# zzuiekongning/MGDT-YOLO

Measured on AMD Instinct MI355X. Metric: images/sec @640x640 bs=32 per GPU, detection forward + NMS (whole job: 1 GPU(s)), higher is better.
Workload: dtype bf16; 1 GPU; mspa_c2f_gd_yolov8-n (MSPA-C2f + GD neck + Detect, nc=80) 640x640 inference, batch 32/GPU: forward + decode + NMS(conf 0.25, iou 0.7), hipGraph replay, 4 batches in flight (one captured graph per resident batch, replayed round-robin on 4 streams); global_batch=32, parallelism=replicas x1 (batch-sharded, no data-path collective), rccl_ranks=1, input=bfloat16 NCHW images, 8 different batches resident in HBM (600 MiB) cycled, detections_last_step=9600, weights=seeded random init (no checkpoints offline), batches_in_flight=4

## Files before the change

mgdt_yolo_amd/csrc/pointwise.hip:

```cpp
#include <algorithm>
#include <vector>

#include <type_traits>
#include "common.h"

#define SPR_SPLITS 16

static inline int grid_for(long work, int block = 256, int cap = 8192) { return (int)std::min<long>((work + block - 1) / block, cap); }

struct PixIdx { FastDiv fq, fw, fh; int Q, W, H; };
static inline PixIdx make_pixidx(int H, int W, int Q) { return PixIdx{make_fastdiv((uint32_t)Q), make_fastdiv((uint32_t)W), make_fastdiv((uint32_t)H), Q, W, H}; }
__device__ __forceinline__ void decode_idx(uint32_t i, const PixIdx& d, int& n, int& h, int& w, int& q) {
  uint32_t t = fdiv(i, d.fq);
  q = (int)(i - t * d.Q);
  uint32_t t2 = fdiv(t, d.fw);
  w = (int)(t - t2 * d.W);
  uint32_t t3 = fdiv(t2, d.fh);
  h = (int)(t2 - t3 * d.H);
  n = (int)t3;
}
template <typename T, int V> __device__ __forceinline__ void ldv(const T* p, float (&v)[V]) {
#pragma unroll
  for (int k = 0; k < V; k += 4) {
    f32x4 t = load4<T>(p + k);
// ... 399 lines not shown
    for (int hj = 0; hj < hid; ++hj) s = fmaf(w2s[ci * r2 + hj], hbuf[gi * hid + hj], s);
    obuf[o] = 1.f / (1.f + expf(-s));
  }
  __syncthreads();
  SPR_STAMP();
  for (int ci = tid; ci < cw; ci += 256) {
    float mx = -INFINITY;
    for (int gi = 0; gi < G; ++gi) mx = fmaxf(mx, obuf[gi * cw + ci]);
    float den = 0.f;
    for (int gi = 0; gi < G; ++gi) { const float e = expf(obuf[gi * cw + ci] - mx); att[gi * cw + ci] = e; den += e; }
    for (int gi = 0; gi < G; ++gi) att[gi * cw + ci] /= den;
  }
  __syncthreads();
}

template <typename T, int V>
__global__ __launch_bounds__(256) void spr_attn_scale_kernel(const float* __restrict__ partial, const float* __restrict__ w1, const float* __restrict__ b1,
                                                             const float* __restrict__ w2, const float* __restrict__ b2, int C, int G, int H, int W,
                                                             const T* __restrict__ x, long xsn, long xsh, long xsw, T* __restrict__ y, long ysn, long ysh,
                                                             long ysw, FastDiv fd_q, FastDiv fd_w, int nsplit, int tiles_x, int tiles_y, SprPool pa, SprPool pb, FastDiv fd_gst,
                                                             FastDiv fd_tx, FastDiv fd_l4, int fast, unsigned long long* dbg) {
  extern __shared__ float sm[];
  unsigned long long TS[10]; int nt = 0;
  auto stamp = [&]() __attribute__((always_inline)) { if (dbg) TS[nt++] = __builtin_amdgcn_s_memrealtime(); };
  stamp();
  const int n = blockIdx.y, cw = C / G, hid = cw / 4;
  float* pooled = sm;
  float* hbuf = sm + C * 5;
  float* obuf = hbuf + G * hid;
  float* att = obuf + C;
  const int hs1 = bin_start(1, H, 2), he0 = bin_end(0, H, 2), ws1 = bin_start(1, W, 2), we0 = bin_end(0, W, 2);
  const float cnt[5] = {(float)H * W, (float)he0 * we0, (float)he0 * (W - ws1), (float)(H - hs1) * we0, (float)(H - hs1) * (W - ws1)};
  __shared__ float red[5 * 256];
  if (fast) {
    spr_prologue_fast(partial, w1, b1, w2, b2, C, G, n, nsplit, tiles_x, tiles_y, fd_gst, fd_tx, fd_l4, cnt, sm, red, att, dbg ? TS : nullptr, nt);
  } else {
    if (tiles_x > 0) {
      const int gst = nsplit / (tiles_x * tiles_y);
      for (int c0 = 0; c0 < C; c0 += 256) {
        const int lanes_c = min(C - c0, 256);
        const int ph = 256 / lanes_c;
        const int c = c0 + threadIdx.x % lanes_c, sp0 = threadIdx.x / lanes_c;
        float acc[5] = {0.f, 0.f, 0.f, 0.f, 0.f};
        if (sp0 < ph) {
          for (int sp = sp0; sp < nsplit; sp += ph) {
            const float v = partial[((long)n * nsplit + sp) * C + c];
            const int tile = sp / gst, ty = tile / tiles_x, tx = tile - ty * tiles_x;
            const int bin = (2 * ty >= tiles_y ? 2 : 0) + (2 * tx >= tiles_x ? 1 : 0);
            acc[0] += v;
            acc[1] += bin == 0 ? v : 0.f;
            acc[2] += bin == 1 ? v : 0.f;
            acc[3] += bin == 2 ? v : 0.f;
            acc[4] += bin == 3 ? v : 0.f;
          }
        }
#pragma unroll
        for (int k = 0; k < 5; ++k) red[k * 256 + threadIdx.x] = acc[k];
        __syncthreads();
        for (int o = threadIdx.x; o < lanes_c * 5; o += 256) {
          const int cc = o % lanes_c, k = o / lanes_c;
          float sum = 0.f;
          for (int p = 0; p < ph; ++p) sum += red[k * 256 + p * lanes_c + cc];
          pooled[(c0 + cc) * 5 + k] = sum / cnt[k];
        }
        __syncthreads();
      }
    } else {
      for (int i = threadIdx.x; i < C * 5; i += 256) {
        float sum = 0.f;
        for (int sp = 0; sp < nsplit; ++sp) sum += partial[((long)n * nsplit + sp) * C * 5 + i];
        pooled[i] = sum / cnt[i % 5];
      }
      __syncthreads();
    }
    for (int o = threadIdx.x; o < G * hid; o += 256) {
      int gi = o / hid, hj = o % hid;
      const float* wr = w1 + (long)hj * 5 * cw;
      float acc = b1[hj];
      for (int c = 0; c < cw; ++c) acc = fmaf(wr[c], pooled[(gi * cw + c) * 5 + 0], acc);
      for (int c = 0; c < cw; ++c)
        for (int bn = 0; bn < 4; ++bn) acc = fmaf(wr[cw + c * 4 + bn], pooled[(gi * cw + c) * 5 + 1 + bn], acc);
      hbuf[o] = fmaxf(acc, 0.f);
    }
    __syncthreads();
    for (int o = threadIdx.x; o < C; o += 256) {
      int gi = o / cw, c = o % cw;
      float acc = b2[c];
      for (int hj = 0; hj < hid; ++hj) acc = fmaf(w2[(long)c * hid + hj], hbuf[gi * hid + hj], acc);
      obuf[o] = 1.f / (1.f + expf(-acc));
    }
    __syncthreads();
    for (int c = threadIdx.x; c < cw; c += 256) {
      float mx = -INFINITY;
      for (int gi = 0; gi < G; ++gi) mx = fmaxf(mx, obuf[gi * cw + c]);
      float den = 0.f;
      for (int gi = 0; gi < G; ++gi) den += expf(obuf[gi * cw + c] - mx);
      for (int gi = 0; gi < G; ++gi) att[gi * cw + c] = expf(obuf[gi * cw + c] - mx) / den;
    }
    __syncthreads();
  }
  stamp();
  auto fin = [&]() __attribute__((always_inline)) { if (dbg) { __builtin_amdgcn_s_waitcnt(0); stamp(); if (threadIdx.x == 0) for (int k = 0; k < 8; ++k) dbg[((size_t)blockIdx.y * gridDim.x + blockIdx.x) * 8 + k] = TS[k]; } };
  {
    const int fa = pa.F, fb = pb.F, fm = max(fa, fb);
    const bool cells = fm > 0 && (fm == 2 || fm == 4) && (fa == 0 || fa == fm || (fm == 4 && fa == 2)) && (fb == 0 || fb == fm || (fm == 4 && fb == 2)) && !(fa == fb);
    if (cells) {
      const SprPool none = {nullptr, 0, 0, 0, 0};
      const SprPool big = fa == fm ? pa : (fb == fm ? pb : none), small = (fa && fa < fm) ? pa : ((fb && fb < fm) ? pb : none);
      if (fm == 4) spr_scale_cells<T, V, 4>(x, xsn, xsh, xsw, y, ysn, ysh, ysw, att, n, H, W, C, big, small);
      else spr_scale_cells<T, V, 2>(x, xsn, xsh, xsw, y, ysn, ysh, ysw, att, n, H, W, C, big, small);
      fin();
      return;
    }
  }
  const int Q = C / V, HW = H * W;
  const int p0 = (int)((long)blockIdx.x * HW / gridDim.x), p1 = (int)((long)(blockIdx.x + 1) * HW / gridDim.x);
  const uint32_t total = (uint32_t)(p1 - p0) * Q;
  auto one = [&](uint32_t i, long& xo, long& yo, int& qv) __attribute__((always_inline)) {
    const int pl = (int)fdiv(i, fd_q), q = (int)i - pl * Q;
    const int p = p0 + pl, h = (int)fdiv((uint32_t)p, fd_w), w = p - h * W;
    xo = n * xsn + h * xsh + w * xsw + q * V; yo = n * ysn + h * ysh + w * ysw + q * V; qv = q * V;
  };
  uint32_t i = threadIdx.x;
  for (; i + 3 * 256 < total; i += 4 * 256) {
    float v[4][V];
    long yo[4];
    int qv[4];
#pragma unroll
    for (int u = 0; u < 4; ++u) { long xo; one(i + u * 256, xo, yo[u], qv[u]); ldv<T, V>(x + xo, v[u]); }
#pragma unroll
    for (int u = 0; u < 4; ++u) {
#pragma unroll
      for (int k = 0; k < V; ++k) v[u][k] *= att[qv[u] + k];
      stv<T, V>(y + yo[u], v[u]);
    }
  }
  for (; i < total; i += 256) {
    long xo, yo; int qv; float v[V];
    one(i, xo, yo, qv);
    ldv<T, V>(x + xo, v);
#pragma unroll
    for (int k = 0; k < V; ++k) v[k] *= att[qv + k];
    stv<T, V>(y + yo, v);
  }
  const SprPool pools[2] = {pa, pb};
#pragma unroll
  for (int pi = 0; pi < 2; ++pi) {
    const SprPool P = pools[pi];
    if (P.F == 0) continue;
    const int F = P.F, Ho = H / F, Wo = W / F, HWo = Ho * Wo;
    const int q0 = (int)((long)blockIdx.x * HWo / gridDim.x), q1 = (int)((long)(blockIdx.x + 1) * HWo / gridDim.x);
    const float inv = 1.f / (float)(F * F);
    for (int j = threadIdx.x; j < (q1 - q0) * Q; j += 256) {
      const int pl = j / Q, q = j - pl * Q, po = q0 + pl, oy = po / Wo, ox = po - oy * Wo;
      float a[V], acc[V];
#pragma unroll
      for (int k = 0; k < V; ++k) { a[k] = att[q * V + k]; acc[k] = 0.f; }
      for (int yy = 0; yy < F; ++yy)
        for (int xx = 0; xx < F; ++xx) {
          float v[V];
          ldv<T, V>(x + n * xsn + (long)(oy * F + yy) * xsh + (long)(ox * F + xx) * xsw + q * V, v);
#pragma unroll
          for (int k = 0; k < V; ++k) acc[k] += (float)(T)(v[k] * a[k]);
        }
#pragma unroll
      for (int k = 0; k < V; ++k) acc[k] *= inv;
      stv<T, V>((T*)P.y + n * P.sn + oy * P.sh + ox * P.sw + q * V, acc);
    }
  }
  fin();
}

extern "C" int mgdt_spr_attn_scale_fwd(const float* pooled, int nsplit, int tiles_x, int tiles_y, const float* fc1_w, const float* fc1_b, const float* fc2_w, const float* fc2_b, int groups,
                                       const mgdt_view* x, const mgdt_view* y, const mgdt_view* pool_a, const mgdt_view* pool_b, int dtype, mgdt_stream s) {
  if (nsplit <= 0) nsplit = SPR_SPLITS;
  if (tiles_x > 0 && (tiles_y <= 0 || nsplit % (tiles_x * tiles_y) || tiles_x % 2 || tiles_y % 2 || x->h % 2 || x->w % 2))
    MGDT_FAIL(MGDT_BAD_SHAPE, "spr_attn_scale: per-tile sums need an even tile grid over an even map (nsplit=%d tiles %dx%d)", nsplit, tiles_y, tiles_x);
  if (!pooled || !fc1_w || !fc1_b || !fc2_w || !fc2_b || !view_ok(x) || !view_ok(y)) MGDT_FAIL(MGDT_BAD_ARG, "spr_attn_scale: null/empty argument");
  const int c = x->c;
  if (groups < 1 || c % groups || (c / groups) % 4 || c > 4096) MGDT_FAIL(MGDT_BAD_SHAPE, "spr_attn_scale: c=%d groups=%d", c, groups);
  if (!vec4_ok(x, dtype) || !vec4_ok(y, dtype) || x->n != y->n || x->h != y->h || x->w != y->w || y->c != c)
    MGDT_FAIL(MGDT_BAD_SHAPE, "spr_attn_scale: views must be matching NHWC, c%%4==0");
  const int cw = c / groups, hid = cw / 4;
  size_t lds = (size_t)(c * 5 + groups * hid + 2 * c) * sizeof(float);
  const size_t wbytes = ((size_t)hid * (5 * cw + 4) + (size_t)cw * (hid + 1) + hid + cw + 4) * sizeof(float);
  const int fast = tiles_x > 0 && c <= 256 && lds + wbytes <= 48 * 1024 && ((uintptr_t)fc1_w & 15) == 0;
  if (fast) lds += wbytes;
  SprPool pl[2] = {{nullptr, 0, 0, 0, 0}, {nullptr, 0, 0, 0, 0}};
  bool pool8 = true;
  const mgdt_view* pv[2] = {pool_a, pool_b};
  for (int i = 0; i < 2; ++i) {
    const mgdt_view* p = pv[i];
    if (!p || !p->p) continue;
    if (!view_ok(p) || !vec4_ok(p, dtype) || p->n != x->n || p->c != c || p->h < 1 || x->h % p->h || x->w % p->w || x->h / p->h != x->w / p->w)
      MGDT_FAIL(MGDT_BAD_SHAPE, "spr_attn_scale: a pooled output must be an NHWC view of the same n, c whose size divides the map by one factor");
    pl[i].y = p->p; pl[i].sn = p->sn; pl[i].sh = p->sh; pl[i].sw = p->sw; pl[i].F = x->h / p->h;
    pool8 = pool8 && vecN_ok(p, dtype, 8);
  }
  static unsigned long long* dbgbuf = nullptr;
  if (getenv("MGDT_SPR_DBG") && !dbgbuf) (void)hipMalloc((void**)&dbgbuf, 4096 * 8 * 8);
  int gK = 0;
  MGDT_DISPATCH_TV(dtype, vecN_ok(x, dtype, 8) && vecN_ok(y, dtype, 8) && pool8, {
    const long vecs = (long)x->h * x->w * (c / V);
    static const long per_wg = getenv("MGDT_SPR_VECS") ? atol(getenv("MGDT_SPR_VECS")) : 2048;
    static const long kmax = getenv("MGDT_SPR_KMAX") ? atol(getenv("MGDT_SPR_KMAX")) : 12;
    const int K = (int)std::max<long>(1, std::min<long>(kmax, vecs / per_wg));
    spr_attn_scale_kernel<T, V><<<dim3(K, x->n), 256, lds, (hipStream_t)s>>>(pooled, fc1_w, fc1_b, fc2_w, fc2_b, c, groups, x->h, x->w, (const T*)x->p, x->sn,
                                                                              x->sh, x->sw, (T*)y->p, y->sn, y->sh, y->sw, make_fastdiv((uint32_t)(c / V)),
                                                                              make_fastdiv((uint32_t)x->w), nsplit, tiles_x, tiles_y, pl[0], pl[1],
                                                                              make_fastdiv((uint32_t)(tiles_x > 0 ? nsplit / (tiles_x * tiles_y) : 1)),
                                                                              make_fastdiv((uint32_t)std::max(tiles_x, 1)), make_fastdiv((uint32_t)(5 * cw / 4)), fast, dbgbuf);
    gK = K;
  });
  MGDT_CHECK_LAUNCH("spr_attn_scale_fwd");
  if (dbgbuf && gK * x->n <= 4096) {
    (void)hipStreamSynchronize((hipStream_t)s);
    std::vector<unsigned long long> h((size_t)gK * x->n * 8);
    (void)hipMemcpy(h.data(), dbgbuf, h.size() * 8, hipMemcpyDeviceToHost);
    unsigned long long t0 = ~0ull, t1 = 0; double ph[7] = {0, 0, 0, 0, 0, 0, 0};
    const int ns = fast ? 8 : 3;
    for (int i = 0; i < gK * x->n; ++i) { t0 = std::min(t0, h[i * 8]); t1 = std::max(t1, h[i * 8 + ns - 1]); for (int k = 0; k + 1 < ns; ++k) ph[k] += (double)(h[i * 8 + k + 1] - h[i * 8 + k]); }
    fprintf(stderr, "spr_attn_scale c %d %dx%d: %d wgs, span %.1f us; mean per wg (us):", c, x->h, x->w, gK * x->n, (t1 - t0) * 0.01);
    for (int k = 0; k + 1 < ns; ++k) fprintf(stderr, " %.2f", ph[k] * 0.01 / (gK * x->n));
    fprintf(stderr, fast ? "  (issue | loads land | sums | fc1 | fc2 | softmax | scale)\n" : "  (prologue | scale)\n");
  }
  return MGDT_OK;
}

template <typename T, int V>
__global__ void scale_channels_kernel(const T* __restrict__ x, long xsn, long xsh, long xsw, const float* __restrict__ attn,
                                      T* __restrict__ y, long ysn, long ysh, long ysw, uint32_t total, int C, PixIdx d) {
  for (uint32_t i = blockIdx.x * blockDim.x + threadIdx.x; i < total; i += gridDim.x * blockDim.x) {
    int n, h, w, q;
    decode_idx(i, d, n, h, w, q);
    float v[V], a[V];
    ldv<T, V>(x + n * xsn + h * xsh + w * xsw + q * V, v);
    ldv<float, V>(attn + (long)n * C + q * V, a);
#pragma unroll
    for (int k = 0; k < V; ++k) v[k] *= a[k];
    stv<T, V>(y + n * ysn + h * ysh + w * ysw + q * V, v);
  }
}

extern "C" int mgdt_scale_channels_fwd(const mgdt_view* x, const float* attn, const mgdt_view* y, int dtype, mgdt_stream s) {
  if (!view_ok(x) || !view_ok(y) || !attn) MGDT_FAIL(MGDT_BAD_ARG, "scale_channels: null/empty argument");
  if (!vec4_ok(x, dtype) || !vec4_ok(y, dtype) || x->n != y->n || x->h != y->h || x->w != y->w || x->c != y->c)
    MGDT_FAIL(MGDT_BAD_SHAPE, "scale_channels: views must be matching NHWC, c%%4==0");
  long tot = (long)x->n * x->h * x->w * x->c;
  if (tot >= 0x7fffffffL) MGDT_FAIL(MGDT_BAD_SHAPE, "scale_channels: too large");
  MGDT_DISPATCH_TV(dtype, vecN_ok(x, dtype, 8) && vecN_ok(y, dtype, 8), {
    PixIdx d = make_pixidx(x->h, x->w, x->c / V);
    uint32_t total = (uint32_t)(tot / V);
    scale_channels_kernel<T, V><<<grid_for(total), 256, 0, (hipStream_t)s>>>((const T*)x->p, x->sn, x->sh, x->sw, attn, (T*)y->p, y->sn, y->sh, y->sw, total, x->c, d);
  });
  MGDT_CHECK_LAUNCH("scale_channels_fwd");
  return MGDT_OK;
}

__device__ __forceinline__ float pool_max(float a, float b) { return __builtin_elementwise_maximum(a, b); }

template <typename T, int SPPF_CG>
__global__ __launch_bounds__(256) void sppf_pool_kernel(const T* __restrict__ x, long xsn, long xsh, long xsw, T* __restrict__ y1, long s1n,
                                                        long s1h, long s1w, T* __restrict__ y2, long s2n, long s2h, long s2w,
                                                        T* __restrict__ y3, long s3n, long s3h, long s3w, int H, int W) {
  extern __shared__ float sm[];
  const int n = blockIdx.x, c0 = blockIdx.y * SPPF_CG, HW = H * W, WP = W + 4, PP = (H + 4) * WP;
  float* A = sm;
  float* Bf = sm + PP * SPPF_CG;
  constexpr int QN = SPPF_CG / 4;
  const f32x4 ninf = {-INFINITY, -INFINITY, -INFINITY, -INFINITY};
  for (int i = threadIdx.x; i < PP * QN; i += 256) {
    const int pp = i / QN, qq = (i % QN) * 4;
    const int hh = pp / WP - 2, ww = pp % WP - 2;
    const bool in = (unsigned)hh < (unsigned)H && (unsigned)ww < (unsigned)W;
    *(f32x4*)(A + pp * SPPF_CG + qq) = in ? load4<T>(x + n * xsn + hh * xsh + ww * xsw + c0 + qq) : ninf;
    *(f32x4*)(Bf + pp * SPPF_CG + qq) = ninf;
  }
  __syncthreads();
  T* outs[3] = {y1, y2, y3};
  const long on[3] = {s1n, s2n, s3n}, oh[3] = {s1h, s2h, s3h}, ow[3] = {s1w, s2w, s3w};
  for (int pass = 0; pass < 3; ++pass) {
    for (int i = threadIdx.x; i < HW * SPPF_CG; i += 256) {
      const int c = i % SPPF_CG, p = i / SPPF_CG, h = p / W, w = p - h * W;
      const int o = ((h + 2) * WP + w + 2) * SPPF_CG + c;
      const float a0 = A[o - 2 * SPPF_CG], a1 = A[o - SPPF_CG], a2 = A[o], a3 = A[o + SPPF_CG], a4 = A[o + 2 * SPPF_CG];
      Bf[o] = pool_max(pool_max(pool_max(a0, a1), pool_max(a2, a3)), a4);
    }
    __syncthreads();
    for (int i = threadIdx.x; i < HW * SPPF_CG; i += 256) {
      const int c = i % SPPF_CG, p = i / SPPF_CG, h = p / W, w = p - h * W;
      const int o = ((h + 2) * WP + w + 2) * SPPF_CG + c, rs = WP * SPPF_CG;
      const float b0 = Bf[o - 2 * rs], b1 = Bf[o - rs], b2 = Bf[o], b3 = Bf[o + rs], b4 = Bf[o + 2 * rs];
      A[o] = pool_max(pool_max(pool_max(b0, b1), pool_max(b2, b3)), b4);
    }
    __syncthreads();
    for (int i = threadIdx.x; i < HW * QN; i += 256) {
      const int p = i / QN, qq = (i % QN) * 4, h = p / W, w = p - h * W;
      store4<T>(outs[pass] + n * on[pass] + h * oh[pass] + w * ow[pass] + c0 + qq, *(const f32x4*)(A + ((h + 2) * WP + w + 2) * SPPF_CG + qq));
    }
  }
}

template <typename T, int V>
__global__ __launch_bounds__(256) void sppf_pool3_kernel(const T* __restrict__ x, long xsn, long xsh, long xsw, T* __restrict__ y1, long s1n, long s1h, long s1w,
                                                         T* __restrict__ y2, long s2n, long s2h, long s2w, T* __restrict__ y3, long s3n, long s3h, long s3w, int H, int W) {
  extern __shared__ __attribute__((aligned(16))) char sm3[];
  const int n = blockIdx.x, c0 = blockIdx.y * V, WP = W + 12, HP = H + 12;
  T* X = (T*)sm3;
  T* R = X + (size_t)H * WP * V;
  float ninf[V];
#pragma unroll
  for (int k = 0; k < V; ++k) ninf[k] = -INFINITY;
  for (int i = threadIdx.x; i < H * WP; i += 256) {
    const int h = i / WP, wp = i - h * WP, w = wp - 6;
    float v[V];
    if ((unsigned)w < (unsigned)W) ldv<T, V>(x + n * xsn + h * xsh + w * xsw + c0, v);
    else {
#pragma unroll
      for (int k = 0; k < V; ++k) v[k] = -INFINITY;
    }
    stv<T, V>(X + (size_t)i * V, v);
  }
  for (int i = threadIdx.x; i < 3 * 12 * W; i += 256) {
    const int pl = i / (12 * W), rem = i - pl * 12 * W, hr = rem / W, w = rem - hr * W;
    const int hp = hr < 6 ? hr : H + hr;
    stv<T, V>(R + ((size_t)(pl * HP + hp) * W + w) * V, ninf);
  }
  __syncthreads();
  for (int i = threadIdx.x; i < H * W; i += 256) {
    const int h = i / W, w = i - h * W;
    const T* row = X + ((size_t)h * WP + w) * V;
    float t[13][V];
#pragma unroll
    for (int j = 0; j < 13; ++j) ldv<T, V>(row + (size_t)j * V, t[j]);
    float m5[V], m9[V], m13[V];
#pragma unroll
    for (int k = 0; k < V; ++k) {
      m5[k] = pool_max(pool_max(pool_max(t[4][k], t[5][k]), pool_max(t[6][k], t[7][k])), t[8][k]);
      m9[k] = pool_max(pool_max(m5[k], pool_max(t[2][k], t[3][k])), pool_max(t[9][k], t[10][k]));
      m13[k] = pool_max(pool_max(m9[k], pool_max(t[0][k], t[1][k])), pool_max(t[11][k], t[12][k]));
    }
    stv<T, V>(R + ((size_t)(0 * HP + h + 6) * W + w) * V, m5);
    stv<T, V>(R + ((size_t)(1 * HP + h + 6) * W + w) * V, m9);
    stv<T, V>(R + ((size_t)(2 * HP + h + 6) * W + w) * V, m13);
  }
  __syncthreads();
  for (int i = threadIdx.x; i < H * W; i += 256) {
    const int h = i / W, w = i - h * W;
    float o[V], t[V];
#pragma unroll
    for (int k = 0; k < V; ++k) o[k] = -INFINITY;
#pragma unroll
    for (int j = 4; j <= 8; ++j) {
      ldv<T, V>(R + ((size_t)(0 * HP + h + j) * W + w) * V, t);
#pragma unroll
      for (int k = 0; k < V; ++k) o[k] = pool_max(o[k], t[k]);
    }
    stv<T, V>(y1 + n * s1n + h * s1h + w * s1w + c0, o);
#pragma unroll
    for (int k = 0; k < V; ++k) o[k] = -INFINITY;
#pragma unroll
    for (int j = 2; j <= 10; ++j) {
      ldv<T, V>(R + ((size_t)(1 * HP + h + j) * W + w) * V, t);
#pragma unroll
      for (int k = 0; k < V; ++k) o[k] = pool_max(o[k], t[k]);
    }
    stv<T, V>(y2 + n * s2n + h * s2h + w * s2w + c0, o);
#pragma unroll
    for (int k = 0; k < V; ++k) o[k] = -INFINITY;
#pragma unroll
    for (int j = 0; j <= 12; ++j) {
      ldv<T, V>(R + ((size_t)(2 * HP + h + j) * W + w) * V, t);
#pragma unroll
      for (int k = 0; k < V; ++k) o[k] = pool_max(o[k], t[k]);
    }
    stv<T, V>(y3 + n * s3n + h * s3h + w * s3w + c0, o);
  }
}

extern "C" int mgdt_sppf_pool_fwd(const mgdt_view* x, const mgdt_view* y1, const mgdt_view* y2, const mgdt_view* y3, int dtype,
                                  mgdt_stream s) {
  if (!view_ok(x) || !view_ok(y1) || !view_ok(y2) || !view_ok(y3)) MGDT_FAIL(MGDT_BAD_ARG, "sppf_pool: null/empty view");
  for (const mgdt_view* v : {x, y1, y2, y3})
    if (!vec4_ok(v, dtype) || v->n != x->n || v->h != x->h || v->w != x->w || v->c != x->c)
      MGDT_FAIL(MGDT_BAD_SHAPE, "sppf_pool: views must be matching NHWC, c%%4==0");
  {
    static const bool old_form = getenv("MGDT_SPPF_CHAINED") != nullptr;
    bool all8 = true;
    for (const mgdt_view* v : {x, y1, y2, y3}) all8 = all8 && vecN_ok(v, dtype, 8);
    const int V3 = (dtype == MGDT_BF16 && all8) ? 8 : 4;
    const size_t lds3 = ((size_t)x->h * (x->w + 12) + (size_t)3 * (x->h + 12) * x->w) * V3 * dtype_size(dtype);
    if (!old_form && lds3 <= 64 * 1024) {
      dim3 grid3(x->n, x->c / V3);
      MGDT_DISPATCH_TV(dtype, all8, {
        sppf_pool3_kernel<T, V><<<grid3, 256, lds3, (hipStream_t)s>>>((const T*)x->p, x->sn, x->sh, x->sw, (T*)y1->p, y1->sn, y1->sh, y1->sw, (T*)y2->p, y2->sn, y2->sh, y2->sw,
                                                                    (T*)y3->p, y3->sn, y3->sh, y3->sw, x->h, x->w);
      });
      MGDT_CHECK_LAUNCH("sppf_pool_fwd");
      return MGDT_OK;
    }
  }
  const long pp = (long)(x->h + 4) * (x->w + 4);
  const int cg = (x->c % 8 == 0 && pp * 8 * 2 * 4 <= 64 * 1024) ? 8 : 4;
  size_t lds = (size_t)pp * cg * 2 * sizeof(float);
  if (lds > 64 * 1024) MGDT_FAIL(MGDT_BAD_SHAPE, "sppf_pool: the %dx%d map does not fit the LDS plane kernel (h*w <= 2048)", x->h, x->w);
  dim3 grid(x->n, x->c / cg);
#define SPPF_L(CG) MGDT_DISPATCH_DTYPE(dtype, (sppf_pool_kernel<T, CG><<<grid, 256, lds, (hipStream_t)s>>>((const T*)x->p, x->sn, x->sh, x->sw, (T*)y1->p, y1->sn, y1->sh, y1->sw, \
                                                 (T*)y2->p, y2->sn, y2->sh, y2->sw, (T*)y3->p, y3->sn, y3->sh, y3->sw, x->h, x->w)))
  if (cg == 8) SPPF_L(8); else SPPF_L(4);
#undef SPPF_L
  MGDT_CHECK_LAUNCH("sppf_pool_fwd");
  return MGDT_OK;
}

template <typename T, int V>
__global__ void avgpool_kernel(const T* __restrict__ x, long xsn, long xsh, long xsw, int H, int W, T* __restrict__ y, long ysn,
                               long ysh, long ysw, uint32_t total, PixIdx d) {
  for (uint32_t i = blockIdx.x * blockDim.x + threadIdx.x; i < total; i += gridDim.x * blockDim.x) {
    int n, oy, ox, q;
    decode_idx(i, d, n, oy, ox, q);
    int y0 = bin_start(oy, H, d.H), y1 = bin_end(oy, H, d.H), x0 = bin_start(ox, W, d.W), x1 = bin_end(ox, W, d.W);
    float acc[V];
#pragma unroll
    for (int k = 0; k < V; ++k) acc[k] = 0.f;
    for (int yy = y0; yy < y1; ++yy)
      for (int xx = x0; xx < x1; ++xx) {
        float v[V];
        ldv<T, V>(x + n * xsn + yy * xsh + xx * xsw + q * V, v);
#pragma unroll
        for (int k = 0; k < V; ++k) acc[k] += v[k];
      }
    float inv = 1.f / (float)((y1 - y0) * (x1 - x0));
#pragma unroll
    for (int k = 0; k < V; ++k) acc[k] *= inv;
    stv<T, V>(y + n * ysn + oy * ysh + ox * ysw + q * V, acc);
  }
}

#define RESAMPLE_ENTRY(fname, kern, label)                                                                                              \
  extern "C" int fname(const mgdt_view* x, const mgdt_view* y, int dtype, mgdt_stream s) {                                             \
    if (!view_ok(x) || !view_ok(y)) MGDT_FAIL(MGDT_BAD_ARG, label ": null/empty view");                                                \
    if (!vec4_ok(x, dtype) || !vec4_ok(y, dtype) || x->n != y->n || x->c != y->c) MGDT_FAIL(MGDT_BAD_SHAPE, label ": NHWC views, c%%4==0, same n/c"); \
    long tot = (long)y->n * y->h * y->w * y->c;                                                                                        \
    if (tot >= 0x7fffffffL) MGDT_FAIL(MGDT_BAD_SHAPE, label ": too large");                                                            \
    MGDT_DISPATCH_TV(dtype, vecN_ok(x, dtype, 8) && vecN_ok(y, dtype, 8), {                                                            \
      PixIdx d = make_pixidx(y->h, y->w, y->c / V);                                                                                    \
      uint32_t total = (uint32_t)(tot / V);                                                                                            \
      kern<T, V><<<grid_for(total), 256, 0, (hipStream_t)s>>>((const T*)x->p, x->sn, x->sh, x->sw, x->h, x->w, (T*)y->p, y->sn, y->sh, y->sw, total, d); \
    });                                                                                                                                \
    MGDT_CHECK_LAUNCH(label);                                                                                                          \
    return MGDT_OK;                                                                                                                    \
  }

struct Lerp { int i0, i1; float l0, l1; };
__device__ __forceinline__ Lerp lerp_of(int o, int isz, int osz) {
  float scale = (float)isz / (float)osz;
  float src = scale * ((float)o + 0.5f) - 0.5f;
  if (src < 0.f) src = 0.f;
  int i0 = (int)src;
  if (i0 > isz - 1) i0 = isz - 1;
  int i1 = i0 + (i0 < isz - 1 ? 1 : 0);
  float l1 = src - (float)i0;
  return Lerp{i0, i1, 1.f - l1, l1};
}

template <typename T, int V, bool HSIG>
__device__ __forceinline__ void bilerp(const T* x, long sh, long sw, Lerp ly, Lerp lx, float (&o)[V]) {
  float v00[V], v01[V], v10[V], v11[V];
  ldv<T, V>(x + ly.i0 * sh + lx.i0 * sw, v00);
  ldv<T, V>(x + ly.i0 * sh + lx.i1 * sw, v01);
  ldv<T, V>(x + ly.i1 * sh + lx.i0 * sw, v10);
  ldv<T, V>(x + ly.i1 * sh + lx.i1 * sw, v11);
#pragma unroll
  for (int k = 0; k < V; ++k) {
    if (HSIG) {
      v00[k] = fminf(fmaxf(v00[k] + 3.f, 0.f), 6.f) / 6.f; v01[k] = fminf(fmaxf(v01[k] + 3.f, 0.f), 6.f) / 6.f;
      v10[k] = fminf(fmaxf(v10[k] + 3.f, 0.f), 6.f) / 6.f; v11[k] = fminf(fmaxf(v11[k] + 3.f, 0.f), 6.f) / 6.f;
    }
    o[k] = (v00[k] * lx.l0 + v01[k] * lx.l1) * ly.l0 + (v10[k] * lx.l0 + v11[k] * lx.l1) * ly.l1;
  }
}

template <typename T, int V>
__global__ void bilinear_kernel(const T* __restrict__ x, long xsn, long xsh, long xsw, int H, int W, T* __restrict__ y, long ysn,
                                long ysh, long ysw, uint32_t total, PixIdx d) {
  for (uint32_t i = blockIdx.x * blockDim.x + threadIdx.x; i < total; i += gridDim.x * blockDim.x) {
    int n, oy, ox, q;
    decode_idx(i, d, n, oy, ox, q);
    float o[V];
    bilerp<T, V, false>(x + n * xsn + q * V, xsh, xsw, lerp_of(oy, H, d.H), lerp_of(ox, W, d.W), o);
    stv<T, V>(y + n * ysn + oy * ysh + ox * ysw + q * V, o);
  }
}

template <typename T, int V>
__global__ void nearest_kernel(const T* __restrict__ x, long xsn, long xsh, long xsw, int H, int W, T* __restrict__ y, long ysn,
                               long ysh, long ysw, uint32_t total, PixIdx d) {
  const float sy = (float)H / (float)d.H, sx = (float)W / (float)d.W;
  for (uint32_t i = blockIdx.x * blockDim.x + threadIdx.x; i < total; i += gridDim.x * blockDim.x) {
    int n, oy, ox, q;
    decode_idx(i, d, n, oy, ox, q);
    int iy = min((int)floorf((float)oy * sy), H - 1), ix = min((int)floorf((float)ox * sx), W - 1);
    float v[V];
    ldv<T, V>(x + n * xsn + iy * xsh + ix * xsw + q * V, v);
    stv<T, V>(y + n * ysn + oy * ysh + ox * ysw + q * V, v);
  }
}

RESAMPLE_ENTRY(mgdt_adaptive_avgpool_fwd, avgpool_kernel, "adaptive_avgpool")
RESAMPLE_ENTRY(mgdt_bilinear_fwd, bilinear_kernel, "bilinear")
RESAMPLE_ENTRY(mgdt_nearest_fwd, nearest_kernel, "nearest")

template <typename T, int V>
__global__ void inject_kernel(const T* __restrict__ loc, long lsn, long lsh, long lsw, const T* __restrict__ ga, long asn, long ash,
                              long asw, const T* __restrict__ gf, long fsn, long fsh, long fsw, int Hg, int Wg, T* __restrict__ y,
                              long ysn, long ysh, long ysw, uint32_t total, PixIdx d, int use_pool) {
  const int H = d.H, W = d.W;
  for (uint32_t i = blockIdx.x * blockDim.x + threadIdx.x; i < total; i += gridDim.x * blockDim.x) {
    int n, oy, ox, q;
    decode_idx(i, d, n, oy, ox, q);
    float l[V], sig[V], feat[V];
    ldv<T, V>(loc + n * lsn + oy * lsh + ox * lsw + q * V, l);
    if (use_pool) {
      int y0 = bin_start(oy, Hg, H), y1 = bin_end(oy, Hg, H), x0 = bin_start(ox, Wg, W), x1 = bin_end(ox, Wg, W);
#pragma unroll
      for (int k = 0; k < V; ++k) sig[k] = feat[k] = 0.f;
      for (int yy = y0; yy < y1; ++yy)
        for (int xx = x0; xx < x1; ++xx) {
          float a[V], f[V];
          ldv<T, V>(ga + n * asn + yy * ash + xx * asw + q * V, a);
          ldv<T, V>(gf + n * fsn + yy * fsh + xx * fsw + q * V, f);
#pragma unroll
          for (int k = 0; k < V; ++k) { sig[k] += a[k]; feat[k] += f[k]; }
        }
      float inv = 1.f / (float)((y1 - y0) * (x1 - x0));
#pragma unroll
      for (int k = 0; k < V; ++k) { sig[k] *= inv; feat[k] *= inv; }
    } else {
      Lerp ly = lerp_of(oy, Hg, H), lx = lerp_of(ox, Wg, W);
      bilerp<T, V, true>(ga + n * asn + q * V, ash, asw, ly, lx, sig);
      bilerp<T, V, false>(gf + n * fsn + q * V, fsh, fsw, ly, lx, feat);
    }
#pragma unroll
    for (int k = 0; k < V; ++k) l[k] = l[k] * sig[k] + feat[k];
    stv<T, V>(y + n * ysn + oy * ysh + ox * ysw + q * V, l);
  }
}

extern "C" int mgdt_inject_fwd(const mgdt_view* local, const mgdt_view* ga, const mgdt_view* gf, const mgdt_view* y, int dtype,
                               mgdt_stream s) {
  if (!view_ok(local) || !view_ok(ga) || !view_ok(gf) || !view_ok(y)) MGDT_FAIL(MGDT_BAD_ARG, "inject: null/empty view");
  bool v8 = true;
  for (const mgdt_view* v : {local, ga, gf, y}) {
    if (!vec4_ok(v, dtype) || v->n != y->n || v->c != y->c) MGDT_FAIL(MGDT_BAD_SHAPE, "inject: NHWC views, c%%4==0, same n/c");
    v8 = v8 && vecN_ok(v, dtype, 8);
  }
  if (local->h != y->h || local->w != y->w || ga->h != gf->h || ga->w != gf->w) MGDT_FAIL(MGDT_BAD_SHAPE, "inject: spatial mismatch");
  int use_pool = local->h < ga->h;
  long tot = (long)y->n * y->h * y->w * y->c;
  if (tot >= 0x7fffffffL) MGDT_FAIL(MGDT_BAD_SHAPE, "inject: too large");
  MGDT_DISPATCH_TV(dtype, v8, {
    PixIdx d = make_pixidx(y->h, y->w, y->c / V);
    uint32_t total = (uint32_t)(tot / V);
    inject_kernel<T, V><<<grid_for(total), 256, 0, (hipStream_t)s>>>((const T*)local->p, local->sn, local->sh, local->sw, (const T*)ga->p, ga->sn, ga->sh, ga->sw,
                                                                     (const T*)gf->p, gf->sn, gf->sh, gf->sw, ga->h, ga->w, (T*)y->p, y->sn, y->sh, y->sw, total, d, use_pool);
  });
  MGDT_CHECK_LAUNCH("inject_fwd");
  return MGDT_OK;
}

template <typename T>
__global__ __launch_bounds__(256) void dwconv7_ln_kernel(const T* __restrict__ x, long xsn, long xsh, long xsw,
                                                         const float* __restrict__ dw, const float* __restrict__ db,
                                                         const float* __restrict__ lw, const float* __restrict__ lb, float eps,
                                                         T* __restrict__ y, long ysn, long ysh, long ysw, int N, int H, int W, int C,
                                                         T* __restrict__ uo = nullptr, long usn = 0, long ush = 0, long usw = 0) {
  const int Q = C / 4, PPB = 256 / Q;
  const int q = threadIdx.x % Q, pl = threadIdx.x / Q;
  const long M = (long)N * H * W;
  const long m = blockIdx.x * (long)PPB + pl;
  const bool active = pl < PPB && m < M;
  __shared__ float red[256];
  f32x4 acc = f32x4{0.f, 0.f, 0.f, 0.f};
  int n = 0, oy = 0, ox = 0;
  if (active) {
    n = (int)(m / ((long)H * W));
    int rem = (int)(m - (long)n * H * W);
    oy = rem / W;
    ox = rem - oy * W;
    acc = *(const f32x4*)(db + q * 4);
    for (int ky = 0; ky < 7; ++ky) {
      int iy = oy + ky - 3;
      if (iy < 0 || iy >= H) continue;
      for (int kx = 0; kx < 7; ++kx) {
        int ix = ox + kx - 3;
        if (ix < 0 || ix >= W) continue;
        f32x4 v = load4<T>(x + n * xsn + iy * xsh + ix * xsw + q * 4);
        f32x4 wv = *(const f32x4*)(dw + (long)(ky * 7 + kx) * C + q * 4);
#pragma unroll
        for (int j = 0; j < 4; ++j) acc[j] = fmaf(v[j], wv[j], acc[j]);
      }
    }
  }
  if (uo && active) store4<T>(uo + n * usn + oy * ush + ox * usw + q * 4, acc);
  red[threadIdx.x] = acc[0] + acc[1] + acc[2] + acc[3];
  __syncthreads();
  float mean = 0.f;
  if (pl < PPB) {
    for (int k = 0; k < Q; ++k) mean += red[pl * Q + k];
    mean /= (float)C;
  }
  __syncthreads();
  f32x4 d = acc - mean;
  red[threadIdx.x] = d[0] * d[0] + d[1] * d[1] + d[2] * d[2] + d[3] * d[3];
  __syncthreads();
  float var = 0.f;
  if (pl < PPB) {
    for (int k = 0; k < Q; ++k) var += red[pl * Q + k];
    var /= (float)C;
  }
  if (active) {
    float rstd = 1.f / sqrtf(var + eps);
    f32x4 g = *(const f32x4*)(lw + q * 4), b = *(const f32x4*)(lb + q * 4);
    store4<T>(y + n * ysn + oy * ysh + ox * ysw + q * 4, d * rstd * g + b);
  }
}

template <typename T, int TS>
__global__ __launch_bounds__(256) void dwconv7_ln_row_kernel(const T* __restrict__ x, long xsn, long xsh, long xsw,
                                                             const float* __restrict__ dw, const float* __restrict__ db,
                                                             const float* __restrict__ lw, const float* __restrict__ lb, float eps,
                                                             T* __restrict__ y, long ysn, long ysh, long ysw, int H, int W, int C,
                                                             T* __restrict__ uo, long usn, long ush, long usw, unsigned long long* dbg) {
  unsigned long long TT[6] = {0, 0, 0, 0, 0, 0};
  const bool dbgw = dbg && threadIdx.x == 0;
  if (dbgw) TT[0] = wall_clock64();
  extern __shared__ __attribute__((aligned(16))) char smem_dw[];
  const int Q = C / 4;
  constexpr int HH = TS + 6, HW_ = TS + 6, NPIX = TS * TS;
  T* halo = (T*)smem_dw;
  float* wl = (float*)(smem_dw + (((size_t)HH * HW_ * C * sizeof(T) + 15) & ~(size_t)15));
  float* red = wl + 49 * C;
  float* stat = red + NPIX * Q;
  const int tiles_x = (W + TS - 1) / TS, tiles_y = (H + TS - 1) / TS;
  const int n = blockIdx.x / (tiles_x * tiles_y), tr = blockIdx.x % (tiles_x * tiles_y);
  const int ty0 = (tr / tiles_x) * TS, tx0 = (tr % tiles_x) * TS;
  const int q = threadIdx.x % Q, row = threadIdx.x / Q;
  constexpr int NST = (HH * HW_ + TS - 1) / TS;
  {
    const long ext = ((long)(H - 1) * xsh + (long)(W - 1) * xsw + C) * (long)sizeof(T);
    const __amdgpu_buffer_rsrc_t rs = __builtin_amdgcn_make_buffer_rsrc((void*)(x + n * xsn), 0, (int)ext, 0x00020000);
    using raw_t = typename std::conditional<sizeof(T) == 2, bf16x4, f32x4>::type;
    raw_t v[NST];
#pragma unroll
    for (int i = 0; i < NST; ++i) {
      const int p = row + i * TS;
      const int hy = p / HW_, hx = p % HW_;
      const int iy = ty0 + hy - 3, ix = tx0 + hx - 3;
      const bool ok = p < HH * HW_ && (unsigned)iy < (unsigned)H && (unsigned)ix < (unsigned)W;
      const uint32_t off = ok ? (uint32_t)((iy * xsh + ix * xsw + q * 4) * (long)sizeof(T)) : 0x80000000u;
      if constexpr (sizeof(T) == 2) v[i] = __builtin_bit_cast(bf16x4, __builtin_amdgcn_raw_buffer_load_b64(rs, off, 0, 0));
      else v[i] = __builtin_bit_cast(f32x4, __builtin_amdgcn_raw_buffer_load_b128(rs, off, 0, 0));
    }
#pragma unroll
    for (int i = 0; i < NST; ++i) {
      const int p = row + i * TS;
      if (p < HH * HW_) *(raw_t*)(halo + (long)p * C + q * 4) = v[i];
    }
  }
  if (dbgw) TT[1] = wall_clock64();
  for (int i = threadIdx.x; i < 49 * Q; i += blockDim.x) *(f32x4*)(wl + i * 4) = *(const f32x4*)(dw + i * 4);
  __syncthreads();
  if (dbgw) TT[2] = wall_clock64();
  f32x4 acc[TS];
  {
    const f32x4 bq = *(const f32x4*)(db + q * 4);
#pragma unroll
    for (int k = 0; k < TS; ++k) acc[k] = bq;
  }
#pragma unroll 1
  for (int ky = 0; ky < 7; ++ky) {
    const T* hrow = halo + (long)(row + ky) * HW_ * C + q * 4;
    f32x4 in[HW_];
#pragma unroll
    for (int i = 0; i < HW_; ++i) in[i] = load4<T>(hrow + i * C);
#pragma unroll
    for (int kx = 0; kx < 7; ++kx) {
      const f32x4 wv = *(const f32x4*)(wl + (ky * 7 + kx) * C + q * 4);
#pragma unroll
      for (int k = 0; k < TS; ++k)
#pragma unroll
        for (int j = 0; j < 4; ++j) acc[k][j] = fmaf(in[k + kx][j], wv[j], acc[k][j]);
    }
  }
  if (dbgw) TT[3] = wall_clock64();
#pragma unroll
  for (int k = 0; k < TS; ++k) red[(row * TS + k) * Q + q] = acc[k][0] + acc[k][1] + acc[k][2] + acc[k][3];
  __syncthreads();
  for (int p = threadIdx.x; p < NPIX; p += blockDim.x) {
    float m = 0.f;
    for (int j = 0; j < Q; ++j) m += red[p * Q + j];
    stat[p] = m / (float)C;
  }
  __syncthreads();
  float mean[TS];
#pragma unroll
  for (int k = 0; k < TS; ++k) {
    mean[k] = stat[row * TS + k];
    const f32x4 d = acc[k] - mean[k];
    red[(row * TS + k) * Q + q] = d[0] * d[0] + d[1] * d[1] + d[2] * d[2] + d[3] * d[3];
  }
  __syncthreads();
  for (int p = threadIdx.x; p < NPIX; p += blockDim.x) {
    float var = 0.f;
    for (int j = 0; j < Q; ++j) var += red[p * Q + j];
    stat[p] = 1.f / sqrtf(var / (float)C + eps);
  }
  __syncthreads();
  if (dbgw) TT[4] = wall_clock64();
  const f32x4 gq = *(const f32x4*)(lw + q * 4), bq2 = *(const f32x4*)(lb + q * 4);
  const int oy = ty0 + row;
  if (oy < H) {
#pragma unroll
    for (int k = 0; k < TS; ++k) {
      const int ox = tx0 + k;
      if (ox >= W) continue;
      const float rstd = stat[row * TS + k];
      if (uo) store4<T>(uo + n * usn + oy * ush + ox * usw + q * 4, acc[k]);
      store4<T>(y + n * ysn + oy * ysh + ox * ysw + q * 4, (acc[k] - mean[k]) * rstd * gq + bq2);
    }
  }
  if (dbgw) { TT[5] = wall_clock64(); for (int i = 0; i < 6; ++i) dbg[blockIdx.x * 6 + i] = TT[i]; }
}

struct DwPlan { int family, ts, nwg, lds, threads; };
static DwPlan dwconv7_ln_plan(int n, int h, int w, int c, int dtype) {
  const int Qt = c / 4;
  auto lds_of = [&](int ts) {
    const size_t halo_b = ((size_t)(ts + 6) * (ts + 6) * c * dtype_size(dtype) + 15) & ~(size_t)15;
    return halo_b + (size_t)49 * c * 4 + (size_t)ts * ts * Qt * 4 + (size_t)ts * ts * sizeof(float);
  };
  auto cost_of = [&](int ts) -> long {
    const size_t l = lds_of(ts);
    if (ts * Qt > 256 || l + 256 > (size_t)(ts == 8 ? 64 : 80) * 1024) return -1;
    const long nwg = (long)n * cdiv(h, ts) * cdiv(w, ts), per_cu = std::max<long>(1, std::min<long>(160 * 1024 / (long)(l + 256), 2048 / (ts * Qt)));
    return cdiv(nwg, 256 * per_cu) * ts * ts;
  };
  static const int force_ts = getenv("MGDT_DW_TS") ? atoi(getenv("MGDT_DW_TS")) : 0;
  const long c8 = cost_of(8), c10 = cost_of(10);
  const int ts = force_ts == 8 || force_ts == 10 ? force_ts : (c10 >= 0 && (c8 < 0 || c10 < c8) ? 10 : 8);
  if (Qt <= 32 && (ts == 8 ? c8 : c10) >= 0)
    return DwPlan{ts == 8 ? MGDT_DW_ROW8 : MGDT_DW_ROW10, ts, n * cdiv(h, ts) * cdiv(w, ts), (int)lds_of(ts), ts * Qt};
  const int PPB = 256 / Qt;
  return DwPlan{MGDT_DW_GENERIC, 0, (int)cdiv((long)n * h * w, (long)PPB), 0, 256};
}

extern "C" int mgdt_dwconv7_ln_route(int n, int h, int w, int c, int dtype, int* out) {
  if (!out) MGDT_FAIL(MGDT_BAD_ARG, "dwconv7_ln_route: null argument");
  if (n < 1 || h < 1 || w < 1 || c < 4 || c % 4 || c > 1024 || (dtype != MGDT_F32 && dtype != MGDT_BF16) || (long)n * h * w >= 0x7fffffffL)
    MGDT_FAIL(MGDT_BAD_SHAPE, "dwconv7_ln_route: n=%d %dx%d c=%d dtype=%d not covered (c%%4==0, c<=1024)", n, h, w, c, dtype);
  const DwPlan p = dwconv7_ln_plan(n, h, w, c, dtype);
  out[0] = p.family; out[1] = p.ts; out[2] = p.nwg; out[3] = p.lds; out[4] = p.threads;
  return MGDT_OK;
}

static int dwconv7_ln_impl(const mgdt_view* x, const float* dw_w, const float* dw_b, const float* ln_w, const float* ln_b, float eps,
                           const mgdt_view* y, const mgdt_view* u, int dtype, mgdt_stream s);
extern "C" int mgdt_dwconv7_ln_fwd(const mgdt_view* x, const float* dw_w, const float* dw_b, const float* ln_w, const float* ln_b,
                                   float eps, const mgdt_view* y, int dtype, mgdt_stream s) {
  return dwconv7_ln_impl(x, dw_w, dw_b, ln_w, ln_b, eps, y, nullptr, dtype, s);
}
extern "C" int mgdt_dwconv7_ln_train_fwd(const mgdt_view* x, const float* dw_w, const float* dw_b, const float* ln_w, const float* ln_b,
                                         float eps, const mgdt_view* y, const mgdt_view* u_out, int dtype, mgdt_stream s) {
  if (!view_ok(u_out) || !vec4_ok(u_out, dtype) || u_out->n != x->n || u_out->h != x->h || u_out->w != x->w || u_out->c != x->c)
    MGDT_FAIL(MGDT_BAD_SHAPE, "dwconv7_ln_train: u_out must be an NHWC view like x");
  return dwconv7_ln_impl(x, dw_w, dw_b, ln_w, ln_b, eps, y, u_out, dtype, s);
}
static int dwconv7_ln_impl(const mgdt_view* x, const float* dw_w, const float* dw_b, const float* ln_w, const float* ln_b, float eps,
                           const mgdt_view* y, const mgdt_view* u, int dtype, mgdt_stream s) {
  if (!view_ok(x) || !view_ok(y) || !dw_w || !dw_b || !ln_w || !ln_b) MGDT_FAIL(MGDT_BAD_ARG, "dwconv7_ln: null/empty argument");
  if (!vec4_ok(x, dtype) || !vec4_ok(y, dtype) || x->n != y->n || x->h != y->h || x->w != y->w || x->c != y->c || x->c / 4 > 256)
    MGDT_FAIL(MGDT_BAD_SHAPE, "dwconv7_ln: matching NHWC views, c%%4==0, c<=1024");
  const DwPlan pl = dwconv7_ln_plan(x->n, x->h, x->w, x->c, dtype);
  if (pl.family != MGDT_DW_GENERIC) {
    const int Qt = x->c / 4, ts = pl.ts, tiles = cdiv(x->h, ts) * cdiv(x->w, ts);
    const size_t lds_t = (size_t)pl.lds;
    static unsigned long long* dbgbuf = nullptr;
    if (getenv("MGDT_DW_DBG") && !dbgbuf) (void)hipMalloc((void**)&dbgbuf, (size_t)x->n * tiles * 6 * 8);
    static std::atomic<bool> attr10_f32{false}, attr10_bf16{false};
    if (ts == 10) {
      MGDT_DISPATCH_DTYPE(dtype, {
        std::atomic<bool>& fl = sizeof(T) == 2 ? attr10_bf16 : attr10_f32;
        if (!fl.load()) {
          (void)hipFuncSetAttribute((const void*)dwconv7_ln_row_kernel<T, 10>, hipFuncAttributeMaxDynamicSharedMemorySize, 80 * 1024);
          fl.store(true);
        }
        dwconv7_ln_row_kernel<T, 10><<<x->n * tiles, 10 * Qt, lds_t, (hipStream_t)s>>>(
            (const T*)x->p, x->sn, x->sh, x->sw, dw_w, dw_b, ln_w, ln_b, eps, (T*)y->p, y->sn, y->sh, y->sw, x->h, x->w, x->c,
            u ? (T*)u->p : nullptr, u ? u->sn : 0, u ? u->sh : 0, u ? u->sw : 0, dbgbuf);
      });
    } else {
      MGDT_DISPATCH_DTYPE(dtype, (dwconv7_ln_row_kernel<T, 8><<<x->n * tiles, 8 * Qt, lds_t, (hipStream_t)s>>>(
                                     (const T*)x->p, x->sn, x->sh, x->sw, dw_w, dw_b, ln_w, ln_b, eps, (T*)y->p, y->sn, y->sh, y->sw, x->h, x->w, x->c,
                                     u ? (T*)u->p : nullptr, u ? u->sn : 0, u ? u->sh : 0, u ? u->sw : 0, dbgbuf)));
    }
    MGDT_CHECK_LAUNCH("dwconv7_ln_fwd(row)");
    if (dbgbuf) {
      const int nwg = x->n * tiles;
      std::vector<unsigned long long> h((size_t)nwg * 6);
      (void)hipStreamSynchronize((hipStream_t)s);
      (void)hipMemcpy(h.data(), dbgbuf, h.size() * 8, hipMemcpyDeviceToHost);
      unsigned long long t0 = ~0ull, t5 = 0; double ph[5] = {0, 0, 0, 0, 0};
      for (int i = 0; i < nwg; ++i) { t0 = std::min(t0, h[i * 6]); t5 = std::max(t5, h[i * 6 + 5]); for (int j = 0; j < 5; ++j) ph[j] += (double)(h[i * 6 + j + 1] - h[i * 6 + j]); }
      fprintf(stderr, "dwconv row x10ns: span %llu; avg per WG: halo %.0f weights+sync %.0f taps %.0f layernorm %.0f store %.0f\n", t5 - t0, ph[0] / nwg, ph[1] / nwg,
// ... 229 lines not shown
```

Before: 41360 images/sec.

## Add specialized 2x bilinear upsample kernel and size SPPF block to map

Adds a dedicated kernel for exact 2x bilinear upsampling. Each thread reads a 3x3 input neighbourhood and writes the four output pixels it covers, and blocks are ordered so each XCD handles a contiguous row range for L2 locality. The generic bilinear path stays available through an env var and for non-2x shapes. Separately, the SPPF pool3 kernel now launches with a block size matched to H*W (up to 1024) instead of a fixed 256, with launch_bounds removed, which may raise register pressure.

```diff
diff --git a/mgdt_yolo_amd/csrc/pointwise.hip b/mgdt_yolo_amd/csrc/pointwise.hip
--- a/mgdt_yolo_amd/csrc/pointwise.hip
+++ b/mgdt_yolo_amd/csrc/pointwise.hip
@@ -725,8 +725,8 @@
 }
 
 template <typename T, int V>
-__global__ __launch_bounds__(256) void sppf_pool3_kernel(const T* __restrict__ x, long xsn, long xsh, long xsw, T* __restrict__ y1, long s1n, long s1h, long s1w,
-                                                         T* __restrict__ y2, long s2n, long s2h, long s2w, T* __restrict__ y3, long s3n, long s3h, long s3w, int H, int W) {
+__global__ void sppf_pool3_kernel(const T* __restrict__ x, long xsn, long xsh, long xsw, T* __restrict__ y1, long s1n, long s1h, long s1w,
+                                  T* __restrict__ y2, long s2n, long s2h, long s2w, T* __restrict__ y3, long s3n, long s3h, long s3w, int H, int W) {
   extern __shared__ __attribute__((aligned(16))) char sm3[];
   const int n = blockIdx.x, c0 = blockIdx.y * V, WP = W + 12, HP = H + 12;
   T* X = (T*)sm3;
@@ -734,7 +734,7 @@
   float ninf[V];
 #pragma unroll
   for (int k = 0; k < V; ++k) ninf[k] = -INFINITY;
-  for (int i = threadIdx.x; i < H * WP; i += 256) {
+  for (int i = threadIdx.x; i < H * WP; i += blockDim.x) {
     const int h = i / WP, wp = i - h * WP, w = wp - 6;
     float v[V];
     if ((unsigned)w < (unsigned)W) ldv<T, V>(x + n * xsn + h * xsh + w * xsw + c0, v);
@@ -744,13 +744,13 @@
     }
     stv<T, V>(X + (size_t)i * V, v);
   }
-  for (int i = threadIdx.x; i < 3 * 12 * W; i += 256) {
+  for (int i = threadIdx.x; i < 3 * 12 * W; i += blockDim.x) {
     const int pl = i / (12 * W), rem = i - pl * 12 * W, hr = rem / W, w = rem - hr * W;
     const int hp = hr < 6 ? hr : H + hr;
     stv<T, V>(R + ((size_t)(pl * HP + hp) * W + w) * V, ninf);
   }
   __syncthreads();
-  for (int i = threadIdx.x; i < H * W; i += 256) {
+  for (int i = threadIdx.x; i < H * W; i += blockDim.x) {
     const int h = i / W, w = i - h * W;
     const T* row = X + ((size_t)h * WP + w) * V;
     float t[13][V];
@@ -768,7 +768,7 @@
     stv<T, V>(R + ((size_t)(2 * HP + h + 6) * W + w) * V, m13);
   }
   __syncthreads();
-  for (int i = threadIdx.x; i < H * W; i += 256) {
+  for (int i = threadIdx.x; i < H * W; i += blockDim.x) {
     const int h = i / W, w = i - h * W;
     float o[V], t[V];
 #pragma unroll
@@ -815,8 +815,9 @@
     const size_t lds3 = ((size_t)x->h * (x->w + 12) + (size_t)3 * (x->h + 12) * x->w) * V3 * dtype_size(dtype);
     if (!old_form && lds3 <= 64 * 1024) {
       dim3 grid3(x->n, x->c / V3);
+      const int threads3 = std::min(1024, (x->h * x->w + 63) / 64 * 64);
       MGDT_DISPATCH_TV(dtype, all8, {
-        sppf_pool3_kernel<T, V><<<grid3, 256, lds3, (hipStream_t)s>>>((const T*)x->p, x->sn, x->sh, x->sw, (T*)y1->p, y1->sn, y1->sh, y1->sw, (T*)y2->p, y2->sn, y2->sh, y2->sw,
+        sppf_pool3_kernel<T, V><<<grid3, threads3, lds3, (hipStream_t)s>>>((const T*)x->p, x->sn, x->sh, x->sw, (T*)y1->p, y1->sn, y1->sh, y1->sw, (T*)y2->p, y2->sn, y2->sh, y2->sw,
                                                                     (T*)y3->p, y3->sn, y3->sh, y3->sw, x->h, x->w);
       });
       MGDT_CHECK_LAUNCH("sppf_pool_fwd");
@@ -860,8 +861,9 @@
   }
 }
 
-#define RESAMPLE_ENTRY(fname, kern, label)                                                                                              \
-  extern "C" int fname(const mgdt_view* x, const mgdt_view* y, int dtype, mgdt_stream s) {                                             \
+#define RESAMPLE_ENTRY(fname, kern, label) extern "C" RESAMPLE_FN(fname, kern, label)
+#define RESAMPLE_FN(fname, kern, label)                                                                                                 \
+  int fname(const mgdt_view* x, const mgdt_view* y, int dtype, mgdt_stream s) {                                                        \
     if (!view_ok(x) || !view_ok(y)) MGDT_FAIL(MGDT_BAD_ARG, label ": null/empty view");                                                \
     if (!vec4_ok(x, dtype) || !vec4_ok(y, dtype) || x->n != y->n || x->c != y->c) MGDT_FAIL(MGDT_BAD_SHAPE, label ": NHWC views, c%%4==0, same n/c"); \
     long tot = (long)y->n * y->h * y->w * y->c;                                                                                        \
@@ -930,9 +932,67 @@
   }
 }
 
+template <typename T, int V>
+__global__ __launch_bounds__(256) void bilinear_up2_kernel(const T* __restrict__ x, long xsn, long xsh, long xsw, T* __restrict__ y, long ysn, long ysh,
+                                                           long ysw, uint32_t per_xcd, uint32_t total, PixIdx d) {
+  const uint32_t v = blockIdx.x, in_xcd = (v >> 3) * 256 + threadIdx.x;
+  const uint32_t i = (v & 7) * per_xcd + in_xcd;
+  if (in_xcd >= per_xcd || i >= total) return;
+  int n, iy, ix, q;
+  decode_idx(i, d, n, iy, ix, q);
+  const int ym = max(iy - 1, 0), yp = min(iy + 1, d.H - 1), xm = max(ix - 1, 0), xp = min(ix + 1, d.W - 1);
+  const float ey0 = iy ? 0.25f : 1.f, ey1 = iy ? 0.75f : 0.f;
+  const float ex0 = ix ? 0.25f : 1.f, ex1 = ix ? 0.75f : 0.f;
+  const T* xb = x + n * xsn + q * V;
+  const T* rows[3] = {xb + ym * xsh, xb + iy * xsh, xb + yp * xsh};
+  const long cols[3] = {xm * xsw, ix * xsw, xp * xsw};
+  float t[3][3][V];
+#pragma unroll
+  for (int r = 0; r < 3; ++r)
+#pragma unroll
+    for (int c = 0; c < 3; ++c) ldv<T, V>(rows[r] + cols[c], t[r][c]);
+  float he[3][V], ho[3][V];
+#pragma unroll
+  for (int r = 0; r < 3; ++r)
+#pragma unroll
+    for (int k = 0; k < V; ++k) {
+      he[r][k] = __fmaf_rn(t[r][0][k], ex0, __fmul_rn(ix ? t[r][1][k] : t[r][2][k], ex1));
+      ho[r][k] = __fmaf_rn(t[r][1][k], 0.75f, __fmul_rn(t[r][2][k], 0.25f));
+    }
+  float o00[V], o01[V], o10[V], o11[V];
+#pragma unroll
+  for (int k = 0; k < V; ++k) {
+    o00[k] = __fmaf_rn(iy ? he[1][k] : he[2][k], ey1, __fmul_rn(he[0][k], ey0));
+    o01[k] = __fmaf_rn(iy ? ho[1][k] : ho[2][k], ey1, __fmul_rn(ho[0][k], ey0));
+    o10[k] = __fmaf_rn(he[2][k], 0.25f, __fmul_rn(he[1][k], 0.75f));
+    o11[k] = __fmaf_rn(ho[2][k], 0.25f, __fmul_rn(ho[1][k], 0.75f));
+  }
+  T* yb = y + n * ysn + (2 * iy) * ysh + (2 * ix) * ysw + q * V;
+  stv<T, V>(yb, o00);
+  stv<T, V>(yb + ysw, o01);
+  stv<T, V>(yb + ysh, o10);
+  stv<T, V>(yb + ysh + ysw, o11);
+}
+
 RESAMPLE_ENTRY(mgdt_adaptive_avgpool_fwd, avgpool_kernel, "adaptive_avgpool")
-RESAMPLE_ENTRY(mgdt_bilinear_fwd, bilinear_kernel, "bilinear")
+static RESAMPLE_FN(bilinear_generic_fwd, bilinear_kernel, "bilinear")
 RESAMPLE_ENTRY(mgdt_nearest_fwd, nearest_kernel, "nearest")
+
+extern "C" int mgdt_bilinear_fwd(const mgdt_view* x, const mgdt_view* y, int dtype, mgdt_stream s) {
+  static const bool generic = getenv("MGDT_BILINEAR_GENERIC") && atoi(getenv("MGDT_BILINEAR_GENERIC")) != 0;
+  const bool up2 = !generic && view_ok(x) && view_ok(y) && y->h == 2 * x->h && y->w == 2 * x->w && vec4_ok(x, dtype) && vec4_ok(y, dtype) && x->n == y->n &&
+                   x->c == y->c && (long)y->n * y->h * y->w * y->c < 0x7fffffffL;
+  if (!up2) return bilinear_generic_fwd(x, y, dtype, s);
+  MGDT_DISPATCH_TV(dtype, vecN_ok(x, dtype, 8) && vecN_ok(y, dtype, 8), {
+    PixIdx d = make_pixidx(x->h, x->w, x->c / V);
+    const long rows = (long)x->n * x->h, row_items = (long)x->w * (x->c / V);
+    const uint32_t per_xcd = (uint32_t)((rows + 7) / 8 * row_items), total = (uint32_t)(rows * row_items);
+    bilinear_up2_kernel<T, V><<<8 * ((per_xcd + 255) / 256), 256, 0, (hipStream_t)s>>>((const T*)x->p, x->sn, x->sh, x->sw, (T*)y->p, y->sn, y->sh, y->sw, per_xcd,
+                                                                                     total, d);
+  });
+  MGDT_CHECK_LAUNCH("bilinear");
+  return MGDT_OK;
+}
 
 template <typename T, int V>
 __global__ void inject_kernel(const T* __restrict__ loc, long lsn, long lsh, long lsw, const T* __restrict__ ga, long asn, long ash,
```

New measurement: 41520 images/sec (median of 6 runs). Within noise of the previous version (+0.4%).
